# facebookresearch/pytorch3d

Hardware: NVIDIA H100
Metric: rasterize frames/sec (fwd+bwd) 512^2 K=8 (higher is better)
Workload: dtype f32

## Files before the change

### pytorch3d_b200/csrc/binning.cuh

```cuda
#pragma once
#include <climits>

#include "common.cuh"
#include "raster_math.cuh"

namespace b200r {

constexpr uint32_t RECT_EMPTY_X = 0x0000FFFFu;

__device__ __forceinline__ void pixel_range(float vmin, float vmax, int S, float range, int& lo, int& hi) {
  const float off = range * 0.5f, scale = (float)S / range, margin = 1e-3f + 1e-6f * (float)S;
  float a = (vmin + off) * scale - 0.5f - margin;
  float b = (vmax + off) * scale - 0.5f + margin;
  a = fminf(fmaxf(a, -1.0f), (float)S + 1.0f);
  b = fminf(fmaxf(b, -2.0f), (float)S);
  lo = max(0, (int)ceilf(a));
  hi = min(S - 1, (int)floorf(b));
}

__device__ __forceinline__ uint2 bbox_to_tile_rect(float xmin, float xmax, float ymin, float ymax, int H, int W,
                                                   float rx, float ry) {
  int ix_lo, ix_hi, iy_lo, iy_hi;
  pixel_range(xmin, xmax, W, rx, ix_lo, ix_hi);
  pixel_range(ymin, ymax, H, ry, iy_lo, iy_hi);
// ... 40 lines not shown
      atomicAdd(tile_count + t, 1 + (__ffs((int)~after) - 1));
    }
    if (++tx > tx1) {
      tx = tx0;
      ++ty;
    }
  }
}

constexpr int ORDER_BITS = 21, ORDER_CLASSES = 3;
__device__ __forceinline__ int order_class(int count, int mean) { return count <= 0 ? 2 : (count > mean ? 0 : 1); }
__device__ __forceinline__ unsigned long long order_key(int count, int mean) {
  return 1ull << (ORDER_BITS * order_class(count, mean));
}

static __global__ void __launch_bounds__(1024) tile_scan_kernel(int* __restrict__ counts, int* __restrict__ offsets, int n,
                                                                int* __restrict__ order) {
  __shared__ long long warp_sums[32];
  __shared__ long long carry_s;
  __shared__ unsigned long long order_sums[32];
  __shared__ unsigned long long order_total, order_carry;
  __shared__ int nonempty_s;
  const int tid = threadIdx.x, lane = tid & 31, wid = tid >> 5;
  if (tid == 0) {
    carry_s = 0;
    nonempty_s = 0;
  }
  pdl_trigger();
  pdl_wait();
  __syncthreads();
  for (int base = 0; base < n; base += 8192) {
    const int i0 = base + tid * 8;
    int v[8];
    const bool vec = i0 + 8 <= n && ((reinterpret_cast<uintptr_t>(counts) | reinterpret_cast<uintptr_t>(offsets)) & 15u) == 0;
    if (vec) {
      const int4 a = *reinterpret_cast<const int4*>(counts + i0), b = *reinterpret_cast<const int4*>(counts + i0 + 4);
// ... 48 lines not shown
    } else {
#pragma unroll
      for (int j = 0; j < 8; ++j)
        if (i0 + j < n) {
          offsets[i0 + j] = o[j];
          counts[i0 + j] = o[j];
        }
    }
    __syncthreads();
    if (tid == 0) carry_s = carry + warp_sums[31];
    __syncthreads();
  }
  if (tid == 0) offsets[n] = (int)min(carry_s, (long long)INT_MAX);
  if (order == nullptr) return;
  __syncthreads();
  const long long total_pairs = carry_s;
  const int mean = (int)min(total_pairs / max(nonempty_s, 1), (long long)INT_MAX);
  unsigned long long mine = 0;
  for (int i = tid; i < n; i += 1024) mine += order_key(offsets[i + 1] - offsets[i], mean);
#pragma unroll
  for (int d = 16; d > 0; d >>= 1) mine += __shfl_xor_sync(0xffffffffu, mine, d);
  if (lane == 0) order_sums[wid] = mine;
  __syncthreads();
  if (tid == 0) {
    unsigned long long t = 0;
    for (int w = 0; w < 32; ++w) t += order_sums[w];
    order_total = t;
    order_carry = 0;
  }
  __syncthreads();
  const unsigned long long total = order_total;
  const unsigned long long fmask = (1ull << ORDER_BITS) - 1;
  long long class_base[ORDER_CLASSES];
  {
    long long at = 0;
#pragma unroll
    for (int c = 0; c < ORDER_CLASSES; ++c) {
      class_base[c] = at;
      at += (long long)((total >> (ORDER_BITS * c)) & fmask);
    }
  }
  for (int base = 0; base < n; base += 8192) {
    const int i0 = base + tid * 8;
    unsigned long long k[8], tot = 0;
#pragma unroll
    for (int j = 0; j < 8; ++j) {
      k[j] = i0 + j < n ? order_key(offsets[i0 + j + 1] - offsets[i0 + j], mean) : 0ull;
      tot += k[j];
    }
    unsigned long long inc = tot;
#pragma unroll
    for (int d = 1; d < 32; d <<= 1) {
      const unsigned long long t = __shfl_up_sync(0xffffffffu, inc, d);
      if (lane >= d) inc += t;
    }
    if (lane == 31) order_sums[wid] = inc;
    __syncthreads();
    if (wid == 0) {
      unsigned long long w = order_sums[lane];
#pragma unroll
      for (int d = 1; d < 32; d <<= 1) {
        const unsigned long long t = __shfl_up_sync(0xffffffffu, w, d);
        if (lane >= d) w += t;
      }
      order_sums[lane] = w;
    }
    __syncthreads();
    unsigned long long excl = order_carry + inc - tot + (wid > 0 ? order_sums[wid - 1] : 0ull);
#pragma unroll
    for (int j = 0; j < 8; ++j) {
      if (i0 + j < n) {
        long long pos = 0;
#pragma unroll
        for (int c = 0; c < ORDER_CLASSES; ++c)
          if (k[j] == (1ull << (ORDER_BITS * c))) pos = class_base[c] + (long long)((excl >> (ORDER_BITS * c)) & fmask);
        order[pos] = i0 + j;
      }
      excl += k[j];
    }
    __syncthreads();
    if (tid == 0) order_carry += order_sums[31];
    __syncthreads();
  }
}

template <bool AGG>
static __global__ void __launch_bounds__(256)
    tile_fill_kernel(const uint4* __restrict__ rect, int64_t E, int TY, int TX, int* __restrict__ cursor,
                     int* __restrict__ pairs, int64_t capacity) {
  const int64_t e = (int64_t)blockIdx.x * blockDim.x + threadIdx.x;
  const int lane = threadIdx.x & 31;
  pdl_trigger();
  pdl_wait();
  uint4 r4 = make_uint4(RECT_EMPTY_X, 0u, 0u, 0u);
  if (e < E) r4 = __ldg(rect + e);
  const uint2 r = make_uint2(r4.x, r4.y);
  const bool empty = rect_empty(r);
  const int n = (int)r4.z;
  const int tx0 = r.x & 0xFFFF, tx1 = r.x >> 16, ty0 = r.y & 0xFFFF, ty1 = r.y >> 16;
  if (!AGG) {
    if (empty) return;
    for (int ty = ty0; ty <= ty1; ++ty)
      for (int tx = tx0; tx <= tx1; ++tx) {
        const int pos = atomicAdd(cursor + (n * TY + ty) * TX + tx, 1);
        if (pos >= 0 && (int64_t)pos < capacity) pairs[pos] = (int)e;
      }
    return;
  }
  const int w = empty ? 1 : tx1 - tx0 + 1;
  const int ntile = empty ? 0 : w * (ty1 - ty0 + 1);
  const int rounds = (int)__reduce_max_sync(0xffffffffu, (unsigned)ntile);
  int tx = tx0, ty = ty0;
  for (int i = 0; i < rounds; ++i) {
    const bool act = i < ntile;
    const int t = act ? (n * TY + ty) * TX + tx : -1 - lane;
    const int tprev = __shfl_up_sync(0xffffffffu, t, 1);
    const bool cont = act && lane > 0 && t == tprev;
    const unsigned conts = __ballot_sync(0xffffffffu, cont);
    const unsigned heads = __ballot_sync(0xffffffffu, act && !cont);
    const int leader = act ? 31 - __clz((int)(heads & (0xffffffffu >> (31 - lane)))) : lane;
    int base = 0;
    if (act && !cont) {
      const unsigned after = lane == 31 ? 0u : conts >> (lane + 1);
      base = atomicAdd(cursor + t, 1 + (__ffs((int)~after) - 1));
    }
    base = __shfl_sync(0xffffffffu, base, leader);
    if (act) {
      const int pos = base + (lane - leader);
      if (pos >= 0 && (int64_t)pos < capacity) pairs[pos] = (int)e;
    }
    if (++tx > tx1) {
      tx = tx0;
      ++ty;
    }
  }
}

#ifndef B200R_BIN_CHUNK
#define B200R_BIN_CHUNK 1024
#endif
constexpr int BIN_CHUNK = B200R_BIN_CHUNK;
constexpr int BIN_MAX_TILES = 8192;

static __global__ void __launch_bounds__(256)
    tile_fill_private_kernel(const uint4* __restrict__ rect, int64_t E, int TY, int TX, int* __restrict__ cursor,
                             int* __restrict__ pairs, int64_t capacity) {
  extern __shared__ int hist[];
  const int tid = threadIdx.x, T = TY * TX;
  const int64_t e0 = (int64_t)blockIdx.x * BIN_CHUNK;
  pdl_trigger();
// ... 140 lines not shown
    sort_sweep<true, NT>(keys, n, k);
    __syncthreads();
    for (int d = k >> 2; d > 0; d >>= 1) {
      sort_sweep<false, NT>(keys, n, d);
      __syncthreads();
    }
  }
  if (in_smem)
    for (int i = threadIdx.x; i < n; i += NT) seg[i] = s_keys[i];
  __syncthreads();
}

struct BinWorkspace {
  int* tile_count;
  int* tile_offset;
  int* tile_order;
  uint4* rect;
  int* pairs;
  int64_t capacity;
  size_t bytes;
};

inline int64_t default_pair_capacity(int64_t E, int N, int H, int W, int tile_h = TILE, int tile_w = TILE) {
  const int64_t tiles = (int64_t)div_up(H, tile_h) * div_up(W, tile_w);
  const int64_t exact = E * tiles;
  const int64_t heur = 32 * E + 64 * (int64_t)N * tiles;
  int64_t c = exact < heur ? exact : heur;
  if (c < 16) c = 16;
  if (c > 0x7fffffff) c = 0x7fffffff;
  return c;
}

inline BinWorkspace carve_workspace(void* base, int64_t E, int N, int H, int W, int64_t capacity, int tile_h = TILE,
                                    int tile_w = TILE) {
  BinWorkspace ws;
  const int64_t ntiles = (int64_t)N * div_up(H, tile_h) * div_up(W, tile_w);
  if (capacity <= 0) capacity = default_pair_capacity(E, N, H, W, tile_h, tile_w);
  ws.capacity = capacity;
  size_t off = 0;
  char* p = static_cast<char*>(base);
  ws.tile_count = reinterpret_cast<int*>(p + off);
  off = align_up(off + sizeof(int) * (size_t)ntiles, 16);
  ws.tile_offset = reinterpret_cast<int*>(p + off);
  off = align_up(off + sizeof(int) * (size_t)(ntiles + 1), 16);
  ws.tile_order = reinterpret_cast<int*>(p + off);
  off = align_up(off + sizeof(int) * (size_t)ntiles, 16);
  ws.rect = reinterpret_cast<uint4*>(p + off);
  off = align_up(off + sizeof(uint4) * (size_t)(E > 0 ? E : 1), 16);
  ws.pairs = reinterpret_cast<int*>(p + off);
  off = align_up(off + sizeof(int) * (size_t)capacity, 16);
  ws.bytes = off;
  return ws;
}

__device__ __forceinline__ unsigned box_pixel_mask(const float4 bx, const float (&col)[8], const float (&row)[4]) {
  unsigned xm = 0, ym = 0;
#pragma unroll
  for (int c = 0; c < 8; ++c) xm |= (!(col[c] > bx.y || col[c] < bx.x) ? 1u : 0u) << c;
#pragma unroll
  for (int r = 0; r < 4; ++r) ym |= (!(row[r] > bx.w || row[r] < bx.z) ? 1u : 0u) << (8 * r);
  return xm * ym;
}

// ... 15 lines not shown
```

### pytorch3d_b200/csrc/raster_meshes.cu

```cuda
#include <cfloat>
#include <climits>
#include <numeric>

#include "binning.cuh"
#include "bulk_copy.cuh"
#include "common.cuh"
#include "raster_math.cuh"

namespace b200r {

constexpr int SETUP_FACES = 256;
#ifndef B200R_MESH_TILE_H
#define B200R_MESH_TILE_H 16
#endif
constexpr int FTW = 16, FTH = B200R_MESH_TILE_H, FTHREADS = FTW * FTH;
static_assert(FTH == 16 || FTH == 8, "16x16 or 16x8 tiles");
constexpr int CHUNK = FTHREADS;
constexpr int SMEMQ_MAX_K = 32;

__device__ __forceinline__ bool face_is_drawable(const Face& f, bool cull_backfaces) {
  const float zmax = fmaxf(fmaxf(f.z0, f.z1), f.z2), zmin = fminf(fminf(f.z0, f.z1), f.z2);
  if (!(zmax >= 0.0f)) return false;
  if ((double)zmin < kEps) return false;
  const float area = edge_fn(f.x0, f.y0, f.x1, f.y1, f.x2, f.y2);
// ... 23 lines not shown
  const bool hi_sure = hi == min(S - 1, (int)floorf(b1)) && b == b;
  if (!lo_sure) {
    while (lo <= hi) {
      const float v = pix_to_ndc(lo, S, range);
      if (!(v > vmax || v < vmin)) break;
      ++lo;
    }
  }
  if (!hi_sure) {
    while (hi >= lo) {
      const float v = pix_to_ndc(hi, S, range);
      if (!(v > vmax || v < vmin)) break;
      --hi;
    }
  }
}

#ifndef B200R_SETUP_CTAS
#define B200R_SETUP_CTAS 1
#endif
template <bool INDEXED>
__global__ void __launch_bounds__(SETUP_FACES, B200R_SETUP_CTAS)
    mesh_setup_count_kernel(const float* __restrict__ face_verts, const float* __restrict__ verts, int64_t V,
                            const int64_t* __restrict__ faces, float* __restrict__ face_verts_out,
                            const int64_t* __restrict__ neighbor, int64_t F, const int64_t* __restrict__ first,
                            const int64_t* __restrict__ num, int N, int H, int W, int TY, int TX, float rx, float ry,
                            float sqrt_blur, int cull_backfaces, uint4* __restrict__ rect,
                            int* __restrict__ tile_count, float4* __restrict__ rec) {
  __shared__ __align__(16) float s_fv[SETUP_FACES * 9];
  __shared__ __align__(8) uint64_t bar;
  const int tid = threadIdx.x;
  const int64_t f0 = (int64_t)blockIdx.x * SETUP_FACES;
  const int nf = (int)min((int64_t)SETUP_FACES, F - f0);
  pdl_trigger();
  if (INDEXED) {
    for (int e = tid; e < nf * 3; e += SETUP_FACES) {
      const int64_t vi = __ldg(faces + f0 * 3 + e);
      const bool ok = vi >= 0 && vi < V;
      const float* v = verts + vi * 3;
      s_fv[e * 3 + 0] = ok ? __ldg(v + 0) : __int_as_float(0x7fc00000);
      s_fv[e * 3 + 1] = ok ? __ldg(v + 1) : __int_as_float(0x7fc00000);
      s_fv[e * 3 + 2] = ok ? __ldg(v + 2) : __int_as_float(0x7fc00000);
    }
    __syncthreads();
    for (int e = tid; e < nf * 9; e += SETUP_FACES) face_verts_out[f0 * 9 + e] = s_fv[e];
  } else {
    if (tid == 0) {
      mbar_init(&bar, 1);
      fence_mbar_init();
    }
    __syncthreads();
    cta_load_words(s_fv, face_verts + f0 * 9, nf * 9, &bar, 0);
  }
  uint2 r = make_uint2(RECT_EMPTY_X, 0u);
  int n = -1;
  const int64_t fi = f0 + tid;
  if (tid < nf) {
    const float* v = s_fv + tid * 9;
    const Face f = {v[0], v[1], v[2], v[3], v[4], v[5], v[6], v[7], v[8]};
    n = find_owner(first, num, N, fi);
    float4 box = make_float4(FLT_MAX, -FLT_MAX, FLT_MAX, -FLT_MAX);
    int4 rng = make_int4(1, 0, 1, 0);
    if (n >= 0 && face_is_drawable(f, cull_backfaces != 0)) {
      face_box(f, sqrt_blur, box.x, box.y, box.z, box.w);
      int ix_lo, ix_hi, iy_lo, iy_hi;
      exact_pixel_range(box.x, box.y, W, rx, ix_lo, ix_hi);
      exact_pixel_range(box.z, box.w, H, ry, iy_lo, iy_hi);
      if (ix_lo <= ix_hi && iy_lo <= iy_hi) {
        rng = make_int4(W - 1 - ix_hi, W - 1 - ix_lo, H - 1 - iy_hi, H - 1 - iy_lo);
        r = make_uint2((uint32_t)(rng.x / FTW) | ((uint32_t)(rng.y / FTW) << 16),
                       (uint32_t)(rng.z / FTH) | ((uint32_t)(rng.w / FTH) << 16));
      }
    }
    rect[fi] = make_uint4(r.x, r.y, (uint32_t)max(n, 0), 0u);
    const int nb = neighbor ? (int)__ldg(neighbor + fi) : -1;
    float4* out = rec + fi * 4;
    out[0] = make_float4(f.x0, f.y0, f.x1, f.y1);
    out[1] = make_float4(f.x2, f.y2, bary_denominator(f), __int_as_float((int)fi));
    out[2] = make_float4(f.z0, f.z1, f.z2, __int_as_float(nb));
    out[3] = sqrt_blur > 0.0f ? box
                              : make_float4(__int_as_float(rng.x), __int_as_float(rng.y), __int_as_float(rng.z),
                                            __int_as_float(rng.w));
  }
  pdl_wait();
  warp_count_rect(r, n, TY, TX, tile_count, tid & 31);
}

struct Hit {
  float z, dist, b0, b1, b2;
};

__device__ __forceinline__ void flag_tie();

template <bool WATCH>
__device__ __forceinline__ bool eval_pixel_face(float px, float py, const Face& f, float den, float blur_radius,
                                                bool persp, bool clip, bool full, float max_z, Hit& h) {
  const float e0 = edge_fn(px, py, f.x1, f.y1, f.x2, f.y2);
  const float e1 = edge_fn(px, py, f.x2, f.y2, f.x0, f.y0);
  const float e2 = edge_fn(px, py, f.x0, f.y0, f.x1, f.y1);
  float w0 = fdiv(e0, den), w1 = fdiv(e1, den), w2 = fdiv(e2, den);
// ... 237 lines not shown
  s.c[slot] = make_float4(fc.z0, fc.z1, fc.z2, __int_as_float(nb));
}

template <typename T>
__device__ __forceinline__ void out_store(T* ptr, const T v) {
  __stcs(ptr, v);
}

struct FineParams {
  const float* face_verts;
  const int64_t* neighbor;
  const float4* rec;
  const int64_t* first;
  const int64_t* num;
  const int* tile_offset;
  const int* tile_order;
  int row_stride;
  int* pairs;
  int64_t capacity;
  int n0;
  int N, H, W, K, TY, TX;
  float rx, ry, blur_radius, sqrt_blur;
  int persp, clip, cull;
  int smem_ints;
  int64_t* pix_to_face;
  float* zbuf;
  float* bary;
  float* dists;
};

// ... 370 lines not shown
  TileWork t;
  int i;
  if (p.tile_order != nullptr) {
    i = p.tile_order[((p.n0 + blockIdx.z) * p.TY + blockIdx.y) * p.TX + blockIdx.x];
    t.tile_x = i % p.TX;
    const int r = i / p.TX;
    t.tile_y = r % p.TY;
    t.n = r / p.TY;
  } else {
    t.tile_x = blockIdx.x;
    t.tile_y = (int)((blockIdx.y * (unsigned)p.row_stride) % (unsigned)p.TY);
    t.n = p.n0 + blockIdx.z;
    i = (t.n * p.TY + t.tile_y) * p.TX + t.tile_x;
  }
  t.seg_begin = p.tile_offset[i];
  const int seg_end = p.tile_offset[i + 1];
  t.overflow = (int64_t)seg_end > p.capacity || seg_end == INT_MAX;
  t.count = t.overflow ? (int)p.num[t.n] : seg_end - t.seg_begin;
  return t;
}

template <bool NB, bool SCAN>
__device__ __forceinline__ int first_walk_order(const TileWork& t) {
  if (t.overflow || NB) return ORDER_INDEX;
  if (SCAN) return ORDER_ARRIVAL;
  return ORDER_INDEX;
}

#ifndef B200R_FINE_CTAS
#define B200R_FINE_CTAS 4
#endif
// ... 197 lines not shown

__global__ void __launch_bounds__(FTHREADS) mesh_fine_bigk_kernel(const FineParams p) {
  __shared__ FaceChunk s;
  const int tid = threadIdx.x, lane = tid & 31;
  const int t = blockIdx.x;
  const int n = t / (p.TY * p.TX);
  const int tile_y = (t / p.TX) % p.TY, tile_x = t % p.TX;
  int xo, yo;
  fthread_pixel(tile_x, tile_y, xo, yo);
  const bool valid = xo < p.W && yo < p.H;
  const float px = pix_to_ndc(p.W - 1 - xo, p.W, p.rx);
  const float py = pix_to_ndc(p.H - 1 - yo, p.H, p.ry);
  const float fx_lo = warp_min(valid ? px : FLT_MAX), fx_hi = warp_max(valid ? px : -FLT_MAX);
  const float fy_lo = warp_min(valid ? py : FLT_MAX), fy_hi = warp_max(valid ? py : -FLT_MAX);
  pdl_wait();
  const int seg_begin = p.tile_offset[t], seg_end = p.tile_offset[t + 1];
  const bool overflow = (int64_t)seg_end > p.capacity || seg_end == INT_MAX;
  const int64_t mesh_first = p.first[n];
  const int count = overflow ? (int)p.num[n] : seg_end - seg_begin;
  const bool persp = p.persp != 0, clip = p.clip != 0, cull = p.cull != 0;
  const int K = p.K;

  if (!overflow && count > 1)
    cta_sort_segment<FTHREADS>(p.pairs + seg_begin, count, reinterpret_cast<int*>(&s),
                               (int)(sizeof(FaceChunk) / sizeof(int)));

  float qz[B200R_MAX_K], qd[B200R_MAX_K];
  int qi[B200R_MAX_K];
  int qn = 0, q_max_idx = -1;
  float q_max_z = -1000.0f;

// ... 334 lines not shown
}

__global__ void __launch_bounds__(256) mesh_gather_kernel(const float* __restrict__ verts, int64_t V,
                                                          const int64_t* __restrict__ faces, int64_t F,
                                                          float* __restrict__ face_verts_out) {
  const int64_t e = (int64_t)blockIdx.x * blockDim.x + threadIdx.x;
  if (e >= F * 3) return;
  const int64_t vi = __ldg(faces + e);
  const bool ok = vi >= 0 && vi < V;
#pragma unroll
  for (int c = 0; c < 3; ++c) face_verts_out[e * 3 + c] = ok ? __ldg(verts + vi * 3 + c) : __int_as_float(0x7fc00000);
}

using namespace b200r;

extern "C" size_t b200r_rasterize_meshes_workspace_bytes(int64_t F, int32_t N, int32_t H, int32_t W,
                                                         int64_t pair_capacity) {
  if (F < 0 || N < 0 || H < 0 || W < 0) return 0;
  return carve_workspace(nullptr, F, N, H, W, pair_capacity, FTH, FTW).bytes +
         FACE_RECORD_BYTES * (size_t)(F > 0 ? F : 1);
}

static int forward_impl(const float* face_verts, const float* verts, int64_t V, const int64_t* faces,
                        float* face_verts_out, int64_t F, const int64_t* first, const int64_t* num,
                        const int64_t* neighbor, int32_t N, int32_t H, int32_t W, float blur_radius, int32_t K,
                        int32_t perspective_correct, int32_t clip_barycentric_coords, int32_t cull_backfaces,
                        int64_t* pix_to_face, float* zbuf, float* bary, float* dists, void* workspace,
                        size_t workspace_bytes, int64_t pair_capacity, void* stream_) {
  cudaStream_t stream = static_cast<cudaStream_t>(stream_);
  if (K > B200R_MAX_K) return fail(B200R_ERR_INVALID_ARGUMENT, "Must have points_per_pixel <= 150");
  if (F < 0 || N < 0 || H < 0 || W < 0 || K < 0) return fail(B200R_ERR_INVALID_ARGUMENT, "negative size");
  if (F > INT_MAX) return fail(B200R_ERR_INVALID_ARGUMENT, "more than 2^31-1 packed faces are not supported");
  if ((int64_t)N * H * W * K == 0) return B200R_OK;
  const int TY = div_up(H, FTH), TX = div_up(W, FTW);
  if (TY > 0xFFFE || TX > 0xFFFE) return fail(B200R_ERR_INVALID_ARGUMENT, "image too large");
  const int64_t ntiles = (int64_t)N * TY * TX;
  if (ntiles > INT_MAX) return fail(B200R_ERR_INVALID_ARGUMENT, "too many tiles");
  BinWorkspace ws = carve_workspace(workspace, F, N, H, W, pair_capacity, FTH, FTW);
  const size_t nrec = (size_t)(F > 0 ? F : 1);
  if (workspace == nullptr || workspace_bytes < ws.bytes + FACE_RECORD_BYTES * nrec)
    return fail(B200R_ERR_WORKSPACE, "workspace too small for rasterize_meshes_forward");
  float4* rec = reinterpret_cast<float4*>(static_cast<char*>(workspace) + ws.bytes);

  const float rx = ndc_range(W, H), ry = ndc_range(H, W);
  const float sqrt_blur = sqrtf(blur_radius);

  const bool prof = profiling_enabled();
  if (prof) phase_timer().record(0, stream);
  zero_ints_kernel<<<(unsigned)((ntiles + 1023) / 1024), 256, 0, stream>>>(ws.tile_count, ntiles);
  B200R_LAUNCHED("zero_ints_kernel");
  if (F > 0) {
    const unsigned sgrid = (unsigned)((F + SETUP_FACES - 1) / SETUP_FACES);
#define B200R_SETUP_LAUNCH(KERNEL, ...) B200R_CUDA_OK(launch_chained(KERNEL, dim3(sgrid), dim3(SETUP_FACES), 0, stream, __VA_ARGS__))
    if (faces != nullptr) {
      B200R_SETUP_LAUNCH(mesh_setup_count_kernel<true>, (const float*)nullptr, verts, V, faces, face_verts_out, neighbor, F,
                         first, num, N, H, W, TY, TX, rx, ry, sqrt_blur, cull_backfaces, ws.rect, ws.tile_count, rec);
      face_verts = face_verts_out;
    } else {
      B200R_SETUP_LAUNCH(mesh_setup_count_kernel<false>, face_verts, (const float*)nullptr, (int64_t)0,
                         (const int64_t*)nullptr, (float*)nullptr, neighbor, F, first, num, N, H, W, TY, TX, rx, ry,
                         sqrt_blur, cull_backfaces, ws.rect, ws.tile_count, rec);
    }
#undef B200R_SETUP_LAUNCH
    B200R_LAUNCHED("mesh_setup_count_kernel");
  }
  int* const tile_order = (blur_radius > 0.0f && ntiles < (1ll << ORDER_BITS)) ? ws.tile_order : nullptr;
  B200R_CUDA_OK(launch_chained(tile_scan_kernel, dim3(1), dim3(1024), 0, stream, ws.tile_count, ws.tile_offset,
                               (int)ntiles, tile_order));
  B200R_LAUNCHED("tile_scan_kernel");
  if (F > 0) {
    B200R_CUDA_OK(launch_chained(tile_fill_kernel<true>, dim3((unsigned)((F + 255) / 256)), dim3(256), 0, stream,
                                 ws.rect, F, TY, TX, ws.tile_count, ws.pairs, ws.capacity));
    B200R_LAUNCHED("tile_fill_kernel");
  }
  if (prof) phase_timer().record(1, stream);
  FineParams p;
  p.face_verts = face_verts;
  p.neighbor = neighbor;
  p.rec = rec;
  p.n0 = 0;
  p.first = first;
  p.num = num;
  p.tile_offset = ws.tile_offset;
  p.tile_order = tile_order;
  p.row_stride = 1;
  if (!(blur_radius > 0.0f)) {
    p.row_stride = (int)(TY * 0.382) | 1;
    while (std::gcd(p.row_stride, TY) != 1) p.row_stride += 2;
  }
  p.pairs = ws.pairs;
  p.capacity = ws.capacity;
  p.N = N; p.H = H; p.W = W; p.K = K; p.TY = TY; p.TX = TX;
  p.rx = rx; p.ry = ry; p.blur_radius = blur_radius; p.sqrt_blur = sqrt_blur;
  p.persp = perspective_correct; p.clip = clip_barycentric_coords; p.cull = cull_backfaces;
  p.smem_ints = 0;
  p.pix_to_face = pix_to_face; p.zbuf = zbuf; p.bary = bary; p.dists = dists;
  const unsigned grid = (unsigned)ntiles;
  const bool no_blur = !(blur_radius > 0.0f);
// ... 168 lines not shown
```

Measured before the change: 18890.

## Fuse mesh setup, counting, scan and fill into one thread-block-cluster binning kernel

Adds a clustered binning path that launches one thread-block cluster per mesh to perform face setup, per-tile counting, offset computation and pair filling in a single kernel, using distributed shared memory and a smem stash of tile rects. This replaces the zero/setup-count/scan/fill kernel chain and the global rect buffer when the image is small enough and there are enough meshes to fill the SMs. The fine rasterizer now reads a separate tile_end array so segments can be non-contiguous, and a standalone tile-order kernel handles the blur case. It adds launch configuration overhead, cluster scheduling constraints and a more complex code path.

```diff
diff --git a/pytorch3d_b200/csrc/binning.cuh b/pytorch3d_b200/csrc/binning.cuh
--- a/pytorch3d_b200/csrc/binning.cuh
+++ b/pytorch3d_b200/csrc/binning.cuh
@@ -78,12 +78,86 @@
   return 1ull << (ORDER_BITS * order_class(count, mean));
 }
 
+template <class Count>
+__device__ __forceinline__ void tile_order_pass(Count cnt, int n, long long total_pairs, int nonempty,
+                                                int* __restrict__ order) {
+  __shared__ unsigned long long order_sums[32];
+  __shared__ unsigned long long order_total, order_carry;
+  const int tid = threadIdx.x, lane = tid & 31, wid = tid >> 5;
+  const int mean = (int)min(total_pairs / max(nonempty, 1), (long long)INT_MAX);
+  unsigned long long mine = 0;
+  for (int i = tid; i < n; i += 1024) mine += order_key(cnt(i), mean);
+#pragma unroll
+  for (int d = 16; d > 0; d >>= 1) mine += __shfl_xor_sync(0xffffffffu, mine, d);
+  if (lane == 0) order_sums[wid] = mine;
+  __syncthreads();
+  if (tid == 0) {
+    unsigned long long t = 0;
+    for (int w = 0; w < 32; ++w) t += order_sums[w];
+    order_total = t;
+    order_carry = 0;
+  }
+  __syncthreads();
+  const unsigned long long total = order_total;
+  const unsigned long long fmask = (1ull << ORDER_BITS) - 1;
+  long long class_base[ORDER_CLASSES];
+  {
+    long long at = 0;
+#pragma unroll
+    for (int c = 0; c < ORDER_CLASSES; ++c) {
+      class_base[c] = at;
+      at += (long long)((total >> (ORDER_BITS * c)) & fmask);
+    }
+  }
+  for (int base = 0; base < n; base += 8192) {
+    const int i0 = base + tid * 8;
+    unsigned long long k[8], tot = 0;
+#pragma unroll
+    for (int j = 0; j < 8; ++j) {
+      k[j] = i0 + j < n ? order_key(cnt(i0 + j), mean) : 0ull;
+      tot += k[j];
+    }
+    unsigned long long inc = tot;
+#pragma unroll
+    for (int d = 1; d < 32; d <<= 1) {
+      const unsigned long long t = __shfl_up_sync(0xffffffffu, inc, d);
+      if (lane >= d) inc += t;
+    }
+    if (lane == 31) order_sums[wid] = inc;
+    __syncthreads();
+    if (wid == 0) {
+      unsigned long long w = order_sums[lane];
+#pragma unroll
+      for (int d = 1; d < 32; d <<= 1) {
+        const unsigned long long t = __shfl_up_sync(0xffffffffu, w, d);
+        if (lane >= d) w += t;
+      }
+      order_sums[lane] = w;
+    }
+    __syncthreads();
+    unsigned long long excl = order_carry + inc - tot + (wid > 0 ? order_sums[wid - 1] : 0ull);
+#pragma unroll
+    for (int j = 0; j < 8; ++j) {
+      if (i0 + j < n) {
+        long long pos = 0;
+#pragma unroll
+        for (int c = 0; c < ORDER_CLASSES; ++c)
+          if (k[j] == (1ull << (ORDER_BITS * c))) pos = class_base[c] + (long long)((excl >> (ORDER_BITS * c)) & fmask);
+        order[pos] = i0 + j;
+      }
+      excl += k[j];
+    }
+    __syncthreads();
+    if (tid == 0) order_carry += order_sums[31];
+    __syncthreads();
+  }
+}
+
+
 static __global__ void __launch_bounds__(1024) tile_scan_kernel(int* __restrict__ counts, int* __restrict__ offsets, int n,
                                                                 int* __restrict__ order) {
   __shared__ long long warp_sums[32];
   __shared__ long long carry_s;
-  __shared__ unsigned long long order_sums[32];
-  __shared__ unsigned long long order_total, order_carry;
   __shared__ int nonempty_s;
   const int tid = threadIdx.x, lane = tid & 31, wid = tid >> 5;
   if (tid == 0) {
@@ -162,99 +236,45 @@
   if (tid == 0) offsets[n] = (int)min(carry_s, (long long)INT_MAX);
   if (order == nullptr) return;
   __syncthreads();
-  const long long total_pairs = carry_s;
-  const int mean = (int)min(total_pairs / max(nonempty_s, 1), (long long)INT_MAX);
-  unsigned long long mine = 0;
-  for (int i = tid; i < n; i += 1024) mine += order_key(offsets[i + 1] - offsets[i], mean);
-#pragma unroll
-  for (int d = 16; d > 0; d >>= 1) mine += __shfl_xor_sync(0xffffffffu, mine, d);
-  if (lane == 0) order_sums[wid] = mine;
-  __syncthreads();
+  tile_order_pass([&](int i) { return offsets[i + 1] - offsets[i]; }, n, carry_s, nonempty_s, order);
+}
+
+static __global__ void __launch_bounds__(1024) tile_order_kernel(const int* __restrict__ counts, int n,
+                                                                 int* __restrict__ order) {
+  __shared__ long long total_s;
+  __shared__ int nonempty_s;
+  const int tid = threadIdx.x;
   if (tid == 0) {
-    unsigned long long t = 0;
-    for (int w = 0; w < 32; ++w) t += order_sums[w];
-    order_total = t;
-    order_carry = 0;
-  }
-  __syncthreads();
-  const unsigned long long total = order_total;
-  const unsigned long long fmask = (1ull << ORDER_BITS) - 1;
-  long long class_base[ORDER_CLASSES];
-  {
-    long long at = 0;
-#pragma unroll
-    for (int c = 0; c < ORDER_CLASSES; ++c) {
-      class_base[c] = at;
-      at += (long long)((total >> (ORDER_BITS * c)) & fmask);
-    }
-  }
-  for (int base = 0; base < n; base += 8192) {
-    const int i0 = base + tid * 8;
-    unsigned long long k[8], tot = 0;
-#pragma unroll
-    for (int j = 0; j < 8; ++j) {
-      k[j] = i0 + j < n ? order_key(offsets[i0 + j + 1] - offsets[i0 + j], mean) : 0ull;
-      tot += k[j];
-    }
-    unsigned long long inc = tot;
-#pragma unroll
-    for (int d = 1; d < 32; d <<= 1) {
-      const unsigned long long t = __shfl_up_sync(0xffffffffu, inc, d);
-      if (lane >= d) inc += t;
-    }
-    if (lane == 31) order_sums[wid] = inc;
-    __syncthreads();
-    if (wid == 0) {
-      unsigned long long w = order_sums[lane];
-#pragma unroll
-      for (int d = 1; d < 32; d <<= 1) {
-        const unsigned long long t = __shfl_up_sync(0xffffffffu, w, d);
-        if (lane >= d) w += t;
-      }
-      order_sums[lane] = w;
-    }
-    __syncthreads();
-    unsigned long long excl = order_carry + inc - tot + (wid > 0 ? order_sums[wid - 1] : 0ull);
-#pragma unroll
-    for (int j = 0; j < 8; ++j) {
-      if (i0 + j < n) {
-        long long pos = 0;
-#pragma unroll
-        for (int c = 0; c < ORDER_CLASSES; ++c)
-          if (k[j] == (1ull << (ORDER_BITS * c))) pos = class_base[c] + (long long)((excl >> (ORDER_BITS * c)) & fmask);
-        order[pos] = i0 + j;
-      }
-      excl += k[j];
-    }
-    __syncthreads();
-    if (tid == 0) order_carry += order_sums[31];
-    __syncthreads();
-  }
-}
-
-template <bool AGG>
-static __global__ void __launch_bounds__(256)
-    tile_fill_kernel(const uint4* __restrict__ rect, int64_t E, int TY, int TX, int* __restrict__ cursor,
-                     int* __restrict__ pairs, int64_t capacity) {
-  const int64_t e = (int64_t)blockIdx.x * blockDim.x + threadIdx.x;
-  const int lane = threadIdx.x & 31;
+    total_s = 0;
+    nonempty_s = 0;
+  }
   pdl_trigger();
   pdl_wait();
-  uint4 r4 = make_uint4(RECT_EMPTY_X, 0u, 0u, 0u);
-  if (e < E) r4 = __ldg(rect + e);
-  const uint2 r = make_uint2(r4.x, r4.y);
+  __syncthreads();
+  long long total = 0;
+  int ne = 0;
+  for (int i = tid; i < n; i += 1024) {
+    const int c = counts[i];
+    total += c;
+    ne += c > 0 ? 1 : 0;
+  }
+#pragma unroll
+  for (int d = 16; d > 0; d >>= 1) {
+    total += __shfl_xor_sync(0xffffffffu, total, d);
+    ne += __shfl_xor_sync(0xffffffffu, ne, d);
+  }
+  if ((tid & 31) == 0) {
+    atomicAdd(reinterpret_cast<unsigned long long*>(&total_s), (unsigned long long)total);
+    atomicAdd(&nonempty_s, ne);
+  }
+  __syncthreads();
+  tile_order_pass([&](int i) { return counts[i]; }, n, total_s, nonempty_s, order);
+}
+
+__device__ __forceinline__ void warp_fill_rect(uint2 r, int n, int TY, int TX, int* __restrict__ cursor,
+                                               int* __restrict__ pairs, int64_t capacity, int e, int lane) {
   const bool empty = rect_empty(r);
-  const int n = (int)r4.z;
   const int tx0 = r.x & 0xFFFF, tx1 = r.x >> 16, ty0 = r.y & 0xFFFF, ty1 = r.y >> 16;
-  if (!AGG) {
-    if (empty) return;
-    for (int ty = ty0; ty <= ty1; ++ty)
-      for (int tx = tx0; tx <= tx1; ++tx) {
-        const int pos = atomicAdd(cursor + (n * TY + ty) * TX + tx, 1);
-        if (pos >= 0 && (int64_t)pos < capacity) pairs[pos] = (int)e;
-      }
-    return;
-  }
   const int w = empty ? 1 : tx1 - tx0 + 1;
   const int ntile = empty ? 0 : w * (ty1 - ty0 + 1);
   const int rounds = (int)__reduce_max_sync(0xffffffffu, (unsigned)ntile);
@@ -275,13 +295,39 @@
     base = __shfl_sync(0xffffffffu, base, leader);
     if (act) {
       const int pos = base + (lane - leader);
-      if (pos >= 0 && (int64_t)pos < capacity) pairs[pos] = (int)e;
+      if (pos >= 0 && (int64_t)pos < capacity) pairs[pos] = e;
     }
     if (++tx > tx1) {
       tx = tx0;
       ++ty;
     }
   }
+}
+
+template <bool AGG>
+static __global__ void __launch_bounds__(256)
+    tile_fill_kernel(const uint4* __restrict__ rect, int64_t E, int TY, int TX, int* __restrict__ cursor,
+                     int* __restrict__ pairs, int64_t capacity) {
+  const int64_t e = (int64_t)blockIdx.x * blockDim.x + threadIdx.x;
+  const int lane = threadIdx.x & 31;
+  pdl_trigger();
+  pdl_wait();
+  uint4 r4 = make_uint4(RECT_EMPTY_X, 0u, 0u, 0u);
+  if (e < E) r4 = __ldg(rect + e);
+  const uint2 r = make_uint2(r4.x, r4.y);
+  const bool empty = rect_empty(r);
+  const int n = (int)r4.z;
+  if (!AGG) {
+    if (empty) return;
+    const int tx0 = r.x & 0xFFFF, tx1 = r.x >> 16, ty0 = r.y & 0xFFFF, ty1 = r.y >> 16;
+    for (int ty = ty0; ty <= ty1; ++ty)
+      for (int tx = tx0; tx <= tx1; ++tx) {
+        const int pos = atomicAdd(cursor + (n * TY + ty) * TX + tx, 1);
+        if (pos >= 0 && (int64_t)pos < capacity) pairs[pos] = (int)e;
+      }
+    return;
+  }
+  warp_fill_rect(r, n, TY, TX, cursor, pairs, capacity, (int)e, lane);
 }
 
 #ifndef B200R_BIN_CHUNK
@@ -452,6 +498,7 @@
 struct BinWorkspace {
   int* tile_count;
   int* tile_offset;
+  int* tile_end;
   int* tile_order;
   uint4* rect;
   int* pairs;
@@ -470,7 +517,7 @@
 }
 
 inline BinWorkspace carve_workspace(void* base, int64_t E, int N, int H, int W, int64_t capacity, int tile_h = TILE,
-                                    int tile_w = TILE) {
+                                    int tile_w = TILE, bool clustered = false) {
   BinWorkspace ws;
   const int64_t ntiles = (int64_t)N * div_up(H, tile_h) * div_up(W, tile_w);
   if (capacity <= 0) capacity = default_pair_capacity(E, N, H, W, tile_h, tile_w);
@@ -481,10 +528,18 @@
   off = align_up(off + sizeof(int) * (size_t)ntiles, 16);
   ws.tile_offset = reinterpret_cast<int*>(p + off);
   off = align_up(off + sizeof(int) * (size_t)(ntiles + 1), 16);
+  ws.tile_end = nullptr;
+  if (clustered) {
+    ws.tile_end = reinterpret_cast<int*>(p + off);
+    off = align_up(off + sizeof(int) * (size_t)ntiles, 16);
+  }
   ws.tile_order = reinterpret_cast<int*>(p + off);
   off = align_up(off + sizeof(int) * (size_t)ntiles, 16);
-  ws.rect = reinterpret_cast<uint4*>(p + off);
-  off = align_up(off + sizeof(uint4) * (size_t)(E > 0 ? E : 1), 16);
+  ws.rect = nullptr;
+  if (!clustered) {
+    ws.rect = reinterpret_cast<uint4*>(p + off);
+    off = align_up(off + sizeof(uint4) * (size_t)(E > 0 ? E : 1), 16);
+  }
   ws.pairs = reinterpret_cast<int*>(p + off);
   off = align_up(off + sizeof(int) * (size_t)capacity, 16);
   ws.bytes = off;
diff --git a/pytorch3d_b200/csrc/raster_meshes.cu b/pytorch3d_b200/csrc/raster_meshes.cu
--- a/pytorch3d_b200/csrc/raster_meshes.cu
+++ b/pytorch3d_b200/csrc/raster_meshes.cu
@@ -1,6 +1,8 @@
 #include <cfloat>
 #include <climits>
 #include <numeric>
+
+#include <cooperative_groups.h>
 
 #include "binning.cuh"
 #include "bulk_copy.cuh"
@@ -8,6 +10,8 @@
 #include "raster_math.cuh"
 
 namespace b200r {
+
+namespace cg = cooperative_groups;
 
 constexpr int SETUP_FACES = 256;
 #ifndef B200R_MESH_TILE_H
@@ -61,6 +65,62 @@
       --hi;
     }
   }
+}
+
+__device__ __forceinline__ int4 box_output_range(float4 box, int H, int W, float rx, float ry) {
+  int ix_lo, ix_hi, iy_lo, iy_hi;
+  exact_pixel_range(box.x, box.y, W, rx, ix_lo, ix_hi);
+  exact_pixel_range(box.z, box.w, H, ry, iy_lo, iy_hi);
+  if (ix_lo <= ix_hi && iy_lo <= iy_hi) return make_int4(W - 1 - ix_hi, W - 1 - ix_lo, H - 1 - iy_hi, H - 1 - iy_lo);
+  return make_int4(1, 0, 1, 0);
+}
+
+__device__ __forceinline__ uint2 range_tile_rect(int4 rng) {
+  if (rng.x > rng.y || rng.z > rng.w) return make_uint2(RECT_EMPTY_X, 0u);
+  return make_uint2((uint32_t)(rng.x / FTW) | ((uint32_t)(rng.y / FTW) << 16),
+                    (uint32_t)(rng.z / FTH) | ((uint32_t)(rng.w / FTH) << 16));
+}
+
+__device__ __forceinline__ uint2 record_tile_rect(float4 r3, int H, int W, float rx, float ry, float sqrt_blur) {
+  if (sqrt_blur > 0.0f) return range_tile_rect(box_output_range(r3, H, W, rx, ry));
+  return range_tile_rect(make_int4(__float_as_int(r3.x), __float_as_int(r3.y), __float_as_int(r3.z), __float_as_int(r3.w)));
+}
+
+__device__ __forceinline__ uint2 setup_face(const float* v, int64_t fi, bool owned, const int64_t* __restrict__ neighbor,
+                                            int H, int W, float rx, float ry, float sqrt_blur, bool cull,
+                                            float4* __restrict__ rec) {
+  const Face f = {v[0], v[1], v[2], v[3], v[4], v[5], v[6], v[7], v[8]};
+  float4 box = make_float4(FLT_MAX, -FLT_MAX, FLT_MAX, -FLT_MAX);
+  int4 rng = make_int4(1, 0, 1, 0);
+  if (owned && face_is_drawable(f, cull)) {
+    face_box(f, sqrt_blur, box.x, box.y, box.z, box.w);
+    rng = box_output_range(box, H, W, rx, ry);
+  }
+  const int nb = neighbor ? (int)__ldg(neighbor + fi) : -1;
+  float4* out = rec + fi * 4;
+  out[0] = make_float4(f.x0, f.y0, f.x1, f.y1);
+  out[1] = make_float4(f.x2, f.y2, bary_denominator(f), __int_as_float((int)fi));
+  out[2] = make_float4(f.z0, f.z1, f.z2, __int_as_float(nb));
+  out[3] = sqrt_blur > 0.0f ? box
+                            : make_float4(__int_as_float(rng.x), __int_as_float(rng.y), __int_as_float(rng.z),
+                                          __int_as_float(rng.w));
+  return range_tile_rect(rng);
+}
+
+template <int NT>
+__device__ __forceinline__ void gather_faces(float* s_fv, const float* __restrict__ verts, int64_t V,
+                                             const int64_t* __restrict__ faces, float* __restrict__ face_verts_out,
+                                             int64_t f0, int nf) {
+  for (int e = threadIdx.x; e < nf * 3; e += NT) {
+    const int64_t vi = __ldg(faces + f0 * 3 + e);
+    const bool ok = vi >= 0 && vi < V;
+    const float* v = verts + vi * 3;
+    s_fv[e * 3 + 0] = ok ? __ldg(v + 0) : __int_as_float(0x7fc00000);
+    s_fv[e * 3 + 1] = ok ? __ldg(v + 1) : __int_as_float(0x7fc00000);
+    s_fv[e * 3 + 2] = ok ? __ldg(v + 2) : __int_as_float(0x7fc00000);
+  }
+  __syncthreads();
+  for (int e = threadIdx.x; e < nf * 9; e += NT) face_verts_out[f0 * 9 + e] = s_fv[e];
 }
 
 #ifndef B200R_SETUP_CTAS
@@ -81,16 +141,7 @@
   const int nf = (int)min((int64_t)SETUP_FACES, F - f0);
   pdl_trigger();
   if (INDEXED) {
-    for (int e = tid; e < nf * 3; e += SETUP_FACES) {
-      const int64_t vi = __ldg(faces + f0 * 3 + e);
-      const bool ok = vi >= 0 && vi < V;
-      const float* v = verts + vi * 3;
-      s_fv[e * 3 + 0] = ok ? __ldg(v + 0) : __int_as_float(0x7fc00000);
-      s_fv[e * 3 + 1] = ok ? __ldg(v + 1) : __int_as_float(0x7fc00000);
-      s_fv[e * 3 + 2] = ok ? __ldg(v + 2) : __int_as_float(0x7fc00000);
-    }
-    __syncthreads();
-    for (int e = tid; e < nf * 9; e += SETUP_FACES) face_verts_out[f0 * 9 + e] = s_fv[e];
+    gather_faces<SETUP_FACES>(s_fv, verts, V, faces, face_verts_out, f0, nf);
   } else {
     if (tid == 0) {
       mbar_init(&bar, 1);
@@ -103,34 +154,168 @@
   int n = -1;
   const int64_t fi = f0 + tid;
   if (tid < nf) {
-    const float* v = s_fv + tid * 9;
-    const Face f = {v[0], v[1], v[2], v[3], v[4], v[5], v[6], v[7], v[8]};
     n = find_owner(first, num, N, fi);
-    float4 box = make_float4(FLT_MAX, -FLT_MAX, FLT_MAX, -FLT_MAX);
-    int4 rng = make_int4(1, 0, 1, 0);
-    if (n >= 0 && face_is_drawable(f, cull_backfaces != 0)) {
-      face_box(f, sqrt_blur, box.x, box.y, box.z, box.w);
-      int ix_lo, ix_hi, iy_lo, iy_hi;
-      exact_pixel_range(box.x, box.y, W, rx, ix_lo, ix_hi);
-      exact_pixel_range(box.z, box.w, H, ry, iy_lo, iy_hi);
-      if (ix_lo <= ix_hi && iy_lo <= iy_hi) {
-        rng = make_int4(W - 1 - ix_hi, W - 1 - ix_lo, H - 1 - iy_hi, H - 1 - iy_lo);
-        r = make_uint2((uint32_t)(rng.x / FTW) | ((uint32_t)(rng.y / FTW) << 16),
-                       (uint32_t)(rng.z / FTH) | ((uint32_t)(rng.w / FTH) << 16));
-      }
-    }
+    r = setup_face(s_fv + tid * 9, fi, n >= 0, neighbor, H, W, rx, ry, sqrt_blur, cull_backfaces != 0, rec);
     rect[fi] = make_uint4(r.x, r.y, (uint32_t)max(n, 0), 0u);
-    const int nb = neighbor ? (int)__ldg(neighbor + fi) : -1;
-    float4* out = rec + fi * 4;
-    out[0] = make_float4(f.x0, f.y0, f.x1, f.y1);
-    out[1] = make_float4(f.x2, f.y2, bary_denominator(f), __int_as_float((int)fi));
-    out[2] = make_float4(f.z0, f.z1, f.z2, __int_as_float(nb));
-    out[3] = sqrt_blur > 0.0f ? box
-                              : make_float4(__int_as_float(rng.x), __int_as_float(rng.y), __int_as_float(rng.z),
-                                            __int_as_float(rng.w));
   }
   pdl_wait();
   warp_count_rect(r, n, TY, TX, tile_count, tid & 31);
+}
+
+#ifndef B200R_BIN_CLUSTER
+#define B200R_BIN_CLUSTER 16
+#endif
+#ifndef B200R_BIN_THREADS
+#define B200R_BIN_THREADS 512
+#endif
+constexpr int BIN_CLUSTER = B200R_BIN_CLUSTER;
+constexpr int BIN_THREADS = B200R_BIN_THREADS;
+static_assert(BIN_MAX_TILES / BIN_CLUSTER <= BIN_THREADS, "a CTA scans at most one tile per thread");
+constexpr size_t BIN_CLUSTER_SMEM = 100 * 1024;
+
+__device__ __forceinline__ void image_pair_region(unsigned long long before, unsigned long long all, unsigned long long w,
+                                                  int64_t capacity, int64_t& lo, int64_t& hi) {
+  lo = (int64_t)((unsigned __int128)capacity * before / all);
+  hi = (int64_t)((unsigned __int128)capacity * (before + w) / all);
+}
+
+template <bool INDEXED>
+__global__ void __launch_bounds__(BIN_THREADS, 1024 / BIN_THREADS)
+    mesh_bin_cluster_kernel(const float* __restrict__ face_verts, const float* __restrict__ verts, int64_t V,
+                            const int64_t* __restrict__ faces, float* __restrict__ face_verts_out,
+                            const int64_t* __restrict__ neighbor, int64_t F, const int64_t* __restrict__ first,
+                            const int64_t* __restrict__ num, int N, int H, int W, int TY, int TX, float rx, float ry,
+                            float sqrt_blur, int cull_backfaces, int stash_cap, float4* __restrict__ rec,
+                            int* __restrict__ tile_begin, int* __restrict__ tile_end, int* __restrict__ tile_count,
+                            int* __restrict__ pairs, int64_t capacity) {
+  extern __shared__ __align__(16) int smem[];
+  __shared__ long long s_warp[BIN_THREADS / 32];
+  __shared__ long long s_cta_total, s_carry;
+  __shared__ unsigned long long s_weight[3];
+  cg::cluster_group cluster = cg::this_cluster();
+  const int tid = threadIdx.x, lane = tid & 31, wid = tid >> 5;
+  const int rank = (int)cluster.block_rank(), n = blockIdx.y, T = TY * TX;
+  int* const hist = smem;
+  float* const s_fv = reinterpret_cast<float*>(smem + ((T + 3) & ~3));
+  uint2* const stash = reinterpret_cast<uint2*>(s_fv + BIN_THREADS * 9);
+  pdl_trigger();
+  for (int t = tid; t < T; t += BIN_THREADS) hist[t] = 0;
+  if (wid == 0) {
+    unsigned long long before = 0, all = 0, mine = 0;
+    for (int m = lane; m < N; m += 32) {
+      const unsigned long long w = 32ull * (unsigned long long)min(max(__ldg(num + m), (int64_t)0), F) + 64ull * T;
+      all += w;
+      before += m < n ? w : 0;
+      mine += m == n ? w : 0;
+    }
+#pragma unroll
+    for (int d = 16; d > 0; d >>= 1) {
+      before += __shfl_xor_sync(0xffffffffu, before, d);
+      all += __shfl_xor_sync(0xffffffffu, all, d);
+      mine += __shfl_xor_sync(0xffffffffu, mine, d);
+    }
+    if (lane == 0) {
+      s_weight[0] = before;
+      s_weight[1] = all;
+      s_weight[2] = mine;
+    }
+  }
+  __syncthreads();
+  const int64_t fb = __ldg(first + n), fe = fb + __ldg(num + n);
+  const int64_t lo_f = min(max(fb, (int64_t)0), F), hi_f = max(min(fe, F), lo_f);
+  const int64_t share = (hi_f - lo_f + BIN_CLUSTER - 1) / BIN_CLUSTER;
+  const int64_t my_lo = min(lo_f + rank * share, hi_f), my_hi = min(my_lo + share, hi_f);
+
+  for (int64_t c0 = my_lo; c0 < my_hi; c0 += BIN_THREADS) {
+    const int nf = (int)min((int64_t)BIN_THREADS, my_hi - c0);
+    if (INDEXED) {
+      gather_faces<BIN_THREADS>(s_fv, verts, V, faces, face_verts_out, c0, nf);
+    } else {
+      for (int e = tid; e < nf * 9; e += BIN_THREADS) s_fv[e] = __ldg(face_verts + c0 * 9 + e);
+    }
+    __syncthreads();
+    uint2 r = make_uint2(RECT_EMPTY_X, 0u);
+    if (tid < nf) {
+      r = setup_face(s_fv + tid * 9, c0 + tid, true, neighbor, H, W, rx, ry, sqrt_blur, cull_backfaces != 0, rec);
+      if (c0 - my_lo + tid < stash_cap) stash[c0 - my_lo + tid] = r;
+    }
+    warp_count_rect(r, 0, TY, TX, hist, lane);
+    __syncthreads();
+  }
+  if (INDEXED) {
+    const int64_t next = n + 1 < N ? min(max(__ldg(first + n + 1), hi_f), F) : F;
+    for (int g = 0; g < 2; ++g) {
+      const int64_t a = g == 0 ? hi_f : 0, b = g == 0 ? next : (n == 0 ? lo_f : 0);
+      const int64_t gshare = (b - a + BIN_CLUSTER - 1) / BIN_CLUSTER;
+      const int64_t ga = min(a + rank * gshare, b), gb = min(ga + gshare, b);
+      for (int64_t c0 = ga; c0 < gb; c0 += BIN_THREADS) {
+        gather_faces<BIN_THREADS>(s_fv, verts, V, faces, face_verts_out, c0, (int)min((int64_t)BIN_THREADS, gb - c0));
+        __syncthreads();
+      }
+    }
+  }
+  cluster.sync();
+
+  const int TT = (T + BIN_CLUSTER - 1) / BIN_CLUSTER, t0 = min(rank * TT, T), nt = min(TT, T - t0);
+  const int t = t0 + tid;
+  const bool own = tid < nt;
+  int c[BIN_CLUSTER];
+  long long tot = 0;
+#pragma unroll
+  for (int j = 0; j < BIN_CLUSTER; ++j) {
+    c[j] = own ? cluster.map_shared_rank(hist, j)[t] : 0;
+    tot += c[j];
+  }
+  long long inc = tot;
+#pragma unroll
+  for (int d = 1; d < 32; d <<= 1) {
+    const long long v = __shfl_up_sync(0xffffffffu, inc, d);
+    if (lane >= d) inc += v;
+  }
+  if (lane == 31) s_warp[wid] = inc;
+  __syncthreads();
+  if (wid == 0) {
+    long long w = lane < BIN_THREADS / 32 ? s_warp[lane] : 0;
+#pragma unroll
+    for (int d = 1; d < 32; d <<= 1) {
+      const long long v = __shfl_up_sync(0xffffffffu, w, d);
+      if (lane >= d) w += v;
+    }
+    if (lane < BIN_THREADS / 32) s_warp[lane] = w;
+    if (lane == BIN_THREADS / 32 - 1) s_cta_total = w;
+  }
+  cluster.sync();
+  if (wid == 0) {
+    long long v = lane < rank ? *cluster.map_shared_rank(&s_cta_total, lane) : 0;
+#pragma unroll
+    for (int d = 16; d > 0; d >>= 1) v += __shfl_xor_sync(0xffffffffu, v, d);
+    if (lane == 0) s_carry = v;
+  }
+  __syncthreads();
+  int64_t region_lo, region_hi;
+  image_pair_region(s_weight[0], s_weight[1], s_weight[2], capacity, region_lo, region_hi);
+  if (own) {
+    const long long begin = region_lo + s_carry + inc - tot + (wid > 0 ? s_warp[wid - 1] : 0), end = begin + tot;
+    const bool over = end > region_hi;
+    const int g = n * T + t;
+    tile_begin[g] = (int)min(begin, (long long)INT_MAX);
+    tile_end[g] = over ? INT_MAX : (int)end;
+    tile_count[g] = (int)min(tot, (long long)INT_MAX);
+    long long at = begin;
+#pragma unroll
+    for (int j = 0; j < BIN_CLUSTER; ++j) {
+      cluster.map_shared_rank(hist, j)[t] = over ? INT_MIN : (int)at;
+      at += c[j];
+    }
+  }
+  cluster.sync();
+
+  for (int64_t c0 = my_lo; c0 < my_hi; c0 += BIN_THREADS) {
+    const int64_t fi = c0 + tid, i = fi - my_lo;
+    uint2 r = make_uint2(RECT_EMPTY_X, 0u);
+    if (fi < my_hi) r = i < stash_cap ? stash[i] : record_tile_rect(rec[fi * 4 + 3], H, W, rx, ry, sqrt_blur);
+    warp_fill_rect(r, 0, TY, TX, hist, pairs, region_hi, (int)fi, lane);
+  }
 }
 
 struct Hit {
@@ -398,6 +583,7 @@
   const int64_t* first;
   const int64_t* num;
   const int* tile_offset;
+  const int* tile_end;
   const int* tile_order;
   int row_stride;
   int* pairs;
@@ -798,7 +984,7 @@
     i = (t.n * p.TY + t.tile_y) * p.TX + t.tile_x;
   }
   t.seg_begin = p.tile_offset[i];
-  const int seg_end = p.tile_offset[i + 1];
+  const int seg_end = p.tile_end[i];
   t.overflow = (int64_t)seg_end > p.capacity || seg_end == INT_MAX;
   t.count = t.overflow ? (int)p.num[t.n] : seg_end - t.seg_begin;
   return t;
@@ -1026,7 +1212,7 @@
   const float fx_lo = warp_min(valid ? px : FLT_MAX), fx_hi = warp_max(valid ? px : -FLT_MAX);
   const float fy_lo = warp_min(valid ? py : FLT_MAX), fy_hi = warp_max(valid ? py : -FLT_MAX);
   pdl_wait();
-  const int seg_begin = p.tile_offset[t], seg_end = p.tile_offset[t + 1];
+  const int seg_begin = p.tile_offset[t], seg_end = p.tile_end[t];
   const bool overflow = (int64_t)seg_end > p.capacity || seg_end == INT_MAX;
   const int64_t mesh_first = p.first[n];
   const int count = overflow ? (int)p.num[n] : seg_end - seg_begin;
@@ -1391,11 +1577,29 @@
 
 using namespace b200r;
 
+static bool use_cluster_binning(int64_t N, int H, int W) {
+  const int64_t tiles = (int64_t)div_up(H, FTH) * div_up(W, FTW);
+  return N <= 65535 && tiles <= BIN_MAX_TILES && 2 * N * BIN_CLUSTER >= num_sms();
+}
+
 extern "C" size_t b200r_rasterize_meshes_workspace_bytes(int64_t F, int32_t N, int32_t H, int32_t W,
                                                          int64_t pair_capacity) {
   if (F < 0 || N < 0 || H < 0 || W < 0) return 0;
-  return carve_workspace(nullptr, F, N, H, W, pair_capacity, FTH, FTW).bytes +
+  return carve_workspace(nullptr, F, N, H, W, pair_capacity, FTH, FTW, use_cluster_binning(N, H, W)).bytes +
          FACE_RECORD_BYTES * (size_t)(F > 0 ? F : 1);
+}
+
+template <bool INDEXED>
+static int configure_cluster_binning() {
+  int dev = 0;
+  B200R_CUDA_OK(cudaGetDevice(&dev));
+  static bool configured[64] = {};
+  if (dev >= 0 && dev < 64 && configured[dev]) return B200R_OK;
+  B200R_CUDA_OK(cudaFuncSetAttribute(mesh_bin_cluster_kernel<INDEXED>, cudaFuncAttributeNonPortableClusterSizeAllowed, 1));
+  B200R_CUDA_OK(cudaFuncSetAttribute(mesh_bin_cluster_kernel<INDEXED>, cudaFuncAttributeMaxDynamicSharedMemorySize,
+                                     (int)BIN_CLUSTER_SMEM));
+  if (dev >= 0 && dev < 64) configured[dev] = true;
+  return B200R_OK;
 }
 
 static int forward_impl(const float* face_verts, const float* verts, int64_t V, const int64_t* faces,
@@ -1413,7 +1617,8 @@
   if (TY > 0xFFFE || TX > 0xFFFE) return fail(B200R_ERR_INVALID_ARGUMENT, "image too large");
   const int64_t ntiles = (int64_t)N * TY * TX;
   if (ntiles > INT_MAX) return fail(B200R_ERR_INVALID_ARGUMENT, "too many tiles");
-  BinWorkspace ws = carve_workspace(workspace, F, N, H, W, pair_capacity, FTH, FTW);
+  const bool clustered = use_cluster_binning(N, H, W);
+  BinWorkspace ws = carve_workspace(workspace, F, N, H, W, pair_capacity, FTH, FTW, clustered);
   const size_t nrec = (size_t)(F > 0 ? F : 1);
   if (workspace == nullptr || workspace_bytes < ws.bytes + FACE_RECORD_BYTES * nrec)
     return fail(B200R_ERR_WORKSPACE, "workspace too small for rasterize_meshes_forward");
@@ -1424,31 +1629,70 @@
 
   const bool prof = profiling_enabled();
   if (prof) phase_timer().record(0, stream);
-  zero_ints_kernel<<<(unsigned)((ntiles + 1023) / 1024), 256, 0, stream>>>(ws.tile_count, ntiles);
-  B200R_LAUNCHED("zero_ints_kernel");
-  if (F > 0) {
-    const unsigned sgrid = (unsigned)((F + SETUP_FACES - 1) / SETUP_FACES);
-#define B200R_SETUP_LAUNCH(KERNEL, ...) B200R_CUDA_OK(launch_chained(KERNEL, dim3(sgrid), dim3(SETUP_FACES), 0, stream, __VA_ARGS__))
+  int* const tile_order = (blur_radius > 0.0f && ntiles < (1ll << ORDER_BITS)) ? ws.tile_order : nullptr;
+  if (clustered) {
+    const size_t fixed = sizeof(int) * (size_t)((TY * TX + 3) & ~3) + sizeof(float) * BIN_THREADS * 9;
+    const int64_t stash_cap = std::min<int64_t>((F + BIN_CLUSTER - 1) / BIN_CLUSTER,
+                                                (int64_t)((BIN_CLUSTER_SMEM - fixed) / sizeof(uint2)));
+    cudaLaunchConfig_t cfg = {};
+    cfg.gridDim = dim3(BIN_CLUSTER, (unsigned)N);
+    cfg.blockDim = dim3(BIN_THREADS);
+    cfg.dynamicSmemBytes = fixed + sizeof(uint2) * (size_t)stash_cap;
+    cfg.stream = stream;
+    cudaLaunchAttribute attr[1];
+    attr[0].id = cudaLaunchAttributeClusterDimension;
+    attr[0].val.clusterDim.x = BIN_CLUSTER;
+    attr[0].val.clusterDim.y = 1;
+    attr[0].val.clusterDim.z = 1;
+    cfg.attrs = attr;
+    cfg.numAttrs = 1;
     if (faces != nullptr) {
-      B200R_SETUP_LAUNCH(mesh_setup_count_kernel<true>, (const float*)nullptr, verts, V, faces, face_verts_out, neighbor, F,
-                         first, num, N, H, W, TY, TX, rx, ry, sqrt_blur, cull_backfaces, ws.rect, ws.tile_count, rec);
+      if (const int rc = configure_cluster_binning<true>()) return rc;
+      B200R_CUDA_OK(cudaLaunchKernelEx(&cfg, mesh_bin_cluster_kernel<true>, (const float*)nullptr, verts, V, faces,
+                                       face_verts_out, neighbor, F, first, num, (int)N, (int)H, (int)W, TY, TX, rx, ry,
+                                       sqrt_blur, (int)cull_backfaces, (int)stash_cap, rec, ws.tile_offset, ws.tile_end,
+                                       ws.tile_count, ws.pairs, ws.capacity));
       face_verts = face_verts_out;
     } else {
-      B200R_SETUP_LAUNCH(mesh_setup_count_kernel<false>, face_verts, (const float*)nullptr, (int64_t)0,
-                         (const int64_t*)nullptr, (float*)nullptr, neighbor, F, first, num, N, H, W, TY, TX, rx, ry,
-                         sqrt_blur, cull_backfaces, ws.rect, ws.tile_count, rec);
-    }
+      if (const int rc = configure_cluster_binning<false>()) return rc;
+      B200R_CUDA_OK(cudaLaunchKernelEx(&cfg, mesh_bin_cluster_kernel<false>, face_verts, (const float*)nullptr,
+                                       (int64_t)0, (const int64_t*)nullptr, (float*)nullptr, neighbor, F, first, num,
+                                       (int)N, (int)H, (int)W, TY, TX, rx, ry, sqrt_blur, (int)cull_backfaces,
+                                       (int)stash_cap, rec, ws.tile_offset, ws.tile_end, ws.tile_count, ws.pairs,
+                                       ws.capacity));
+    }
+    B200R_LAUNCHED("mesh_bin_cluster_kernel");
+    if (tile_order != nullptr) {
+      B200R_CUDA_OK(launch_chained(tile_order_kernel, dim3(1), dim3(1024), 0, stream, (const int*)ws.tile_count,
+                                   (int)ntiles, tile_order));
+      B200R_LAUNCHED("tile_order_kernel");
+    }
+  } else {
+    zero_ints_kernel<<<(unsigned)((ntiles + 1023) / 1024), 256, 0, stream>>>(ws.tile_count, ntiles);
+    B200R_LAUNCHED("zero_ints_kernel");
+    if (F > 0) {
+      const unsigned sgrid = (unsigned)((F + SETUP_FACES - 1) / SETUP_FACES);
+#define B200R_SETUP_LAUNCH(KERNEL, ...) B200R_CUDA_OK(launch_chained(KERNEL, dim3(sgrid), dim3(SETUP_FACES), 0, stream, __VA_ARGS__))
+      if (faces != nullptr) {
+        B200R_SETUP_LAUNCH(mesh_setup_count_kernel<true>, (const float*)nullptr, verts, V, faces, face_verts_out, neighbor, F,
+                           first, num, N, H, W, TY, TX, rx, ry, sqrt_blur, cull_backfaces, ws.rect, ws.tile_count, rec);
+        face_verts = face_verts_out;
+      } else {
+        B200R_SETUP_LAUNCH(mesh_setup_count_kernel<false>, face_verts, (const float*)nullptr, (int64_t)0,
+                           (const int64_t*)nullptr, (float*)nullptr, neighbor, F, first, num, N, H, W, TY, TX, rx, ry,
+                           sqrt_blur, cull_backfaces, ws.rect, ws.tile_count, rec);
+      }
 #undef B200R_SETUP_LAUNCH
-    B200R_LAUNCHED("mesh_setup_count_kernel");
-  }
-  int* const tile_order = (blur_radius > 0.0f && ntiles < (1ll << ORDER_BITS)) ? ws.tile_order : nullptr;
-  B200R_CUDA_OK(launch_chained(tile_scan_kernel, dim3(1), dim3(1024), 0, stream, ws.tile_count, ws.tile_offset,
-                               (int)ntiles, tile_order));
-  B200R_LAUNCHED("tile_scan_kernel");
-  if (F > 0) {
-    B200R_CUDA_OK(launch_chained(tile_fill_kernel<true>, dim3((unsigned)((F + 255) / 256)), dim3(256), 0, stream,
-                                 ws.rect, F, TY, TX, ws.tile_count, ws.pairs, ws.capacity));
-    B200R_LAUNCHED("tile_fill_kernel");
+      B200R_LAUNCHED("mesh_setup_count_kernel");
+    }
+    B200R_CUDA_OK(launch_chained(tile_scan_kernel, dim3(1), dim3(1024), 0, stream, ws.tile_count, ws.tile_offset,
+                                 (int)ntiles, tile_order));
+    B200R_LAUNCHED("tile_scan_kernel");
+    if (F > 0) {
+      B200R_CUDA_OK(launch_chained(tile_fill_kernel<true>, dim3((unsigned)((F + 255) / 256)), dim3(256), 0, stream,
+                                   ws.rect, F, TY, TX, ws.tile_count, ws.pairs, ws.capacity));
+      B200R_LAUNCHED("tile_fill_kernel");
+    }
   }
   if (prof) phase_timer().record(1, stream);
   FineParams p;
@@ -1459,6 +1703,7 @@
   p.first = first;
   p.num = num;
   p.tile_offset = ws.tile_offset;
+  p.tile_end = clustered ? ws.tile_end : ws.tile_offset + 1;
   p.tile_order = tile_order;
   p.row_stride = 1;
   if (!(blur_radius > 0.0f)) {
```

Measured after the change: 18080, median of 6. 4.3% lower.
